# hsinnan75/Dart

Hardware: AMD Instinct MI355X
Metric: M paired-end reads/sec (2x101 bp vs GRCh38-sized index), host to host; records bit-identical to CPU dart (higher is better)
Workload: dtype u64/u8 integer

## Files before the change

dart_amd/csrc/dg_api.hip:

```cpp
#include "../../include/dartgpu.h"
#include "dg_common.h"
#include "dg_fm.h"
#include "dg_seedq.h"
#include "dg_chain.h"
#include "dg_report.h"
#include "dg_pair.h"
#include "dg_reseed.h"
#include "dg_sort.h"
#include "dg_samfmt.h"
#include <stdio.h>
#include <stdlib.h>
#include <string.h>
#include <string>
#include <algorithm>
#include <vector>
#include <atomic>
#include <mutex>
#include <chrono>
#include <thread>
#include <condition_variable>
#include <fcntl.h>
#include <unistd.h>
#include <sys/stat.h>

// ... 282 lines not shown
{
    if (!c->env_blocking_sync || !c->ev_wait) return hipStreamSynchronize(c->stream);
    const hipError_t e = hipEventRecord(c->ev_wait, c->stream);
    return e != hipSuccess ? e : hipEventSynchronize(c->ev_wait);
}

#ifdef DG_PROFILE_CLASSES
__device__ unsigned long long g_class_cycles[DG_COST_CLASSES + 1], g_class_chunks[DG_COST_CLASSES + 1];
#endif
template <int MINW>
__global__ void __launch_bounds__(64, MINW)
k_report(const DIndex ix, const DParams pr, int n_reads, int paired, const unsigned char *__restrict__ seq,
         const uint32_t *__restrict__ seq_off, const uint16_t *__restrict__ rlen, const uint32_t *__restrict__ seed_off,
         const DJob *__restrict__ jobs, DCand *__restrict__ cands,
         const uint32_t *__restrict__ rep_off, DSeed *__restrict__ work, const unsigned long long *__restrict__ items,
         const uint32_t *__restrict__ n_items_p, dg_report_out *__restrict__ reports, uint32_t *cigpool, uint32_t cigcap,
         unsigned int *tops, unsigned char *ws, const WSLayout L, unsigned long long *ctr, int *err)
{
    const unsigned long long t_wave0 = wall_clock64();
    const int lane = blockIdx.x * blockDim.x + threadIdx.x;
    __shared__ uint32_t lds_pm[64 * PM_LDS_WORDS];
    if (*err >= DG_ABORT) return;
    LaneCtx cx;
#ifdef DG_PROFILE_CLASSES
    __shared__ unsigned long long ph_acc[DG_NCLS * DG_NPHASE], cls_acc[2 * DG_NCLS];
    for (int q = threadIdx.x; q < DG_NCLS * DG_NPHASE; q += 64) ph_acc[q] = 0;
    for (int q = threadIdx.x; q < 2 * DG_NCLS; q += 64) cls_acc[q] = 0;
    __syncthreads();
    cx.ph = ph_acc;
#endif
    cx.lds = lds_pm + (threadIdx.x & 63) * PM_LDS_WORDS;
    cx.ix = &ix; cx.pr = &pr; cx.L = &L;
    cx.ws = ws + (size_t)lane * L.stride;
    cx.n_nw = cx.nw_cells = cx.n_reseed = cx.reseed_w = 0;
    const unsigned int lo = 0u, hi = *n_items_p;
    unsigned int *next = tops + TOP_REPORT_MAIN;
    while (true) {
        unsigned int ticket = 0;
        if ((threadIdx.x & 63) == 0) ticket = atomicAdd(next, 1u);
        ticket = (unsigned int)__shfl((int)ticket, 0, 64);
        const unsigned int base = lo + ticket * 64u;
        if (base >= hi) break;
        const unsigned int idx = base + (threadIdx.x & 63);
        const bool valid = idx < hi;
        const unsigned long long item = valid ? items[idx] : 0ull;
        const int r = (int)(item >> 32);
        const uint32_t ci = (uint32_t)item, rep_i = valid ? rep_off[r] + (ci - seed_off[r]) : 0u;
        DRead rd;
        rd.sub_score = 0; rd.mis_num = 0; rd.mapq = 0;
        cx.seq = seq + seq_off[r]; cx.rlen = rlen[r];
#ifdef DG_PROFILE_CLASSES
        const long long t_begin = clock64();
        cx.cls = (int)(cands[(uint32_t)items[base]].final_n & 31); cx.t_last = t_begin;
#endif
        d_gen_mapping_report(cx, valid, paired ? (r & 1) == 0 : true, rd, cands + ci, valid ? 1 : 0, jobs, work,
                             reports + rep_i, rep_i, cigpool, tops + 0, cigcap, err, 0, 1, true);
#ifdef DG_PROFILE_CLASSES
        if ((threadIdx.x & 63) == 0) { cls_acc[cx.cls] += (unsigned long long)(clock64() - t_begin); cls_acc[DG_NCLS + cx.cls] += 1ull; }
#endif
    }
#ifdef DG_PROFILE_CLASSES
    __syncthreads();
    for (int q = threadIdx.x; q < DG_NCLS * DG_NPHASE; q += 64) if (ph_acc[q]) atomicAdd(&g_phase[q / DG_NPHASE][q % DG_NPHASE], ph_acc[q]);
    if (threadIdx.x < DG_NCLS && cls_acc[DG_NCLS + threadIdx.x]) { atomicAdd(&g_class_cycles[threadIdx.x], cls_acc[threadIdx.x]); atomicAdd(&g_class_chunks[threadIdx.x], cls_acc[DG_NCLS + threadIdx.x]); }
#endif
    d_wave_add(ctr + CTR_NW, cx.n_nw);
    d_wave_add(ctr + CTR_NWCELLS, cx.nw_cells);
// ... 604 lines not shown
    k_unpack<<<(unsigned)((nw + 255) / 256), 256, 0, c->stream>>>(c->packed_in.p, (uint32_t)nw, W2, 1.0 / (double)W2, rlen_all, rlen ? c->rlen.p : nullptr, c->seq.p, c->seq_off.p, c->rlen.p, c->enc.p, c->d_input_bad);
    if (n_n) {
        k_unpack_n<<<(unsigned)((n_n + 255) / 256), 256, 0, c->stream>>>(c->nlist_in.p, (uint32_t)n_n, W2, (uint32_t)(nw * 16), c->seq.p, c->enc.p, c->d_input_bad);
        HIPCHK(hipMemcpyAsync(&c->h_tail->input_bad, c->d_input_bad, 4, hipMemcpyDeviceToHost, c->stream));
    } else c->h_tail->input_bad = 0;
    HIPCHK(hipGetLastError());
    return DG_OK;
}

extern "C" int dg_batch_upload_packed(dg_ctx *c, int n_reads, int rlen_all, const uint16_t *rlen, int words_per_read, const uint32_t *words, const uint32_t *nlist, size_t n_n)
{
    const int rc = enqueue_upload_packed(c, n_reads, rlen_all, rlen, words_per_read, words, nlist, n_n);
    if (rc) return rc;
    HIPCHK(hipStreamSynchronize(c->stream));
    return DG_OK;
}

extern "C" void *dg_host_alloc(size_t bytes)
{
    void *p = nullptr;
    return hipHostMalloc(&p, bytes ? bytes : 1, hipHostMallocDefault) == hipSuccess ? p : nullptr;
}
extern "C" void dg_host_free(void *p) { if (p) (void)hipHostFree(p); }

static WSLayout make_ws_layout(int R)
{
    WSLayout L;
    auto al = [](uint32_t x) { return (x + 15u) & ~15u; };
    uint32_t o = 0;
    const uint32_t nmax = 2u * (uint32_t)R + 32u;
    L.max_rlen = (uint32_t)R;
    L.cig_off = o; L.cig_cap = 4u * (uint32_t)R + 64u; o = al(o + L.cig_cap * 4u);
    L.nwbits_off = o; L.nwbits_words = ((uint32_t)R + 1u) * ((nmax + 7u) / 8u); o = al(o + L.nwbits_words * 4u);
    L.rows_off = o; L.row_cap = (uint32_t)R + 8u; o = al(o + 2u * L.row_cap * 4u);
    L.str_off = o; L.str_cap = al(3u * (uint32_t)R + 64u); o = al(o + 6u * L.str_cap);
    L.kmer_off = o; L.kmer_cap = (uint32_t)R + 8u > 48u ? (uint32_t)R + 8u : 48u; o = al(o + L.kmer_cap * 8u);
    uint32_t rd = 64; while (rd < (uint32_t)R + 1u) rd <<= 1;
    L.ring_diag = rd; L.ring_words = ((uint32_t)R + 64u) / 64u; L.ring_off = o; o = al(o + rd * L.ring_words * 8u);
    L.stride = (o + 255u) & ~255u;
    return L;
}

#define DG_MAX_DEVICES 64
static std::mutex g_lds_mu;
static size_t g_lds_set[2][DG_MAX_DEVICES];
static hipError_t raise_dynamic_lds(const void *fn, int which, int device, size_t lds)
{
    std::lock_guard<std::mutex> lk(g_lds_mu);
    size_t &cur = g_lds_set[which][device & (DG_MAX_DEVICES - 1)];
    if (lds <= cur) return hipSuccess;
    const hipError_t e = hipFuncSetAttribute(fn, hipFuncAttributeMaxDynamicSharedMemorySize, (int)lds);
    if (e == hipSuccess) cur = lds;
    return e;
}

static hipError_t launch_seed(dg_ctx *c, int n, int H, hipEvent_t after_encode = nullptr)
{
    const int W = 2 * ((c->max_rlen + 15) / 16 > 0 ? (c->max_rlen + 15) / 16 : 1);
    hipError_t e = c->enc.ensure((size_t)W * n + 16);
    if (e != hipSuccess) return e;
    int lg = 0;
    while ((1 << lg) < W / 2) lg++;
    if (!c->enc_ready) k_encode<<<(unsigned)((((size_t)n << lg) + 255) / 256), 256, 0, c->stream>>>(c->seq.p, c->seq_off.p, c->rlen.p, n, W, lg, c->enc.p);
    if (after_encode) { e = hipEventRecord(after_encode, c->stream); if (e != hipSuccess) return e; }
    if ((e = c->seed_heavy.ensure((size_t)n + 16)) != hipSuccess) return e;
    unsigned blocks = (unsigned)c->n_cu * (unsigned)c->env_seed_waves;
// ... 791 lines not shown
        k_chain_rules<<<c->n_cu * 4, 64, 0, c->stream>>>(0, c->seed_off.p, c->cands.p, c->ncand.p, c->heavy.p, c->d_tops + TOP_HEAVY_UNITS, c->chain_picks.p, c->chain_todo.p, c->d_err);
        const TileScan ts = make_tile_scan(c, scan_tiles_seed(n), c->d_tops + TOP_TICKET_PAIR, 2);
        k_pair<false><<<(unsigned)((n + PU_THREADS - 1) / PU_THREADS), PU_THREADS, 0, c->stream>>>(
            c->ix, c->pr, n, 0, 0, 1, c->seq.p, c->seq_off.p, c->enc.p, 1, c->rlen.p, c->seed_off.p, c->seeds.p, c->cands.p, c->ncand.p, c->rep_off.p,
            c->slow_units.p, c->reads_out.p, c->reports.p, c->cigfinal.p, 0xFFFFFFFFu, 0xFFFFFFFFu, ts, c->d_sizes, c->d_tops + TOP_CIG, c->d_ctr, c->d_err, CompactOut{nullptr, nullptr, nullptr, nullptr});
        HIPCHK(hipGetLastError());
        k_batch_end<<<1, 256, 0, c->stream>>>(c->d_sizes, c->d_err, c->d_tops, c->d_ctr, c->h_tail);
        HIPCHK(hipGetLastError());
        c->state_zeroed = true;
        HIPCHK(hipStreamSynchronize(c->stream));
        total = c->h_tail->sizes.total_seeds;
        if (c->h_tail->err == DG_E_SEEDS && attempt < 3) { c->cap_seeds = (size_t)total + total / 4 + 1024; continue; }
        if (c->h_tail->err) { snprintf(c->err, 512, "dg_probe_seeds: device status %d", c->h_tail->err); return DG_ERR_INTERNAL; }
        break;
    }
    if (used) *used = total;
    if (total > cap) return DG_ERR_CAPACITY;
    std::vector<SKey> h(total);
    HIPCHK(hipMemcpyAsync(seed_off, c->seed_off.p, ((size_t)n + 1) * 4, hipMemcpyDeviceToHost, c->stream));
    if (total) HIPCHK(hipMemcpyAsync(h.data(), c->seeds.p, (size_t)total * sizeof(SKey), hipMemcpyDeviceToHost, c->stream));
    HIPCHK(hipStreamSynchronize(c->stream));
    for (uint32_t i = 0; i < total; i++) { rpos[i] = sk_rpos(h[i]); slen[i] = sk_rlen(h[i]); gpos[i] = sk_gpos(h[i]); }
    return DG_OK;
}

__global__ void __launch_bounds__(64)
k_probe_nw(int n, const uint32_t *a_off, const uint32_t *b_off, const char *a, const char *b, const uint32_t *out_off,
           uint32_t *out_len, char *out_a, char *out_b, unsigned char *ws, const WSLayout L, const DIndex ix, const DParams pr)
{
    const int i = blockIdx.x * blockDim.x + threadIdx.x;
    if (i >= n) return;
    LaneCtx cx;
    cx.ix = &ix; cx.pr = &pr; cx.L = &L; cx.ws = ws + (size_t)i * L.stride; cx.seq = nullptr; cx.rlen = 0; cx.lds = nullptr;
    cx.n_nw = cx.nw_cells = cx.n_reseed = cx.reseed_w = 0;
    out_len[i] = (uint32_t)d_nw(cx, a + a_off[i], (int)(a_off[i + 1] - a_off[i]), b + b_off[i], (int)(b_off[i + 1] - b_off[i]), out_a + out_off[i], out_b + out_off[i]);
}
__global__ void __launch_bounds__(64)
k_probe_nw_strips(int n, const uint32_t *a_off, const uint32_t *b_off, const char *a, const char *b, const uint32_t *out_off,
                  uint32_t *out_len, char *out_a, char *out_b, const DIndex ix, const DParams pr)
{
    __shared__ uint32_t lds_pm[64 * PM_LDS_WORDS];
    const int i = blockIdx.x * blockDim.x + threadIdx.x;
    if (i >= n) return;
    LaneCtx cx;
    cx.ix = &ix; cx.pr = &pr; cx.L = nullptr; cx.ws = nullptr; cx.seq = nullptr; cx.rlen = 0; cx.lds = lds_pm + (threadIdx.x & 63) * PM_LDS_WORDS;
    cx.n_nw = cx.nw_cells = cx.n_reseed = cx.reseed_w = 0;
    const char *pa = a + a_off[i], *pb = b + b_off[i];
    const int m = (int)(a_off[i + 1] - a_off[i]), nn = (int)(b_off[i + 1] - b_off[i]);
    uint64_t w[6] = {0, 0, 0, 0, 0, 0};
    for (int k = 0; k < m; k++) w[k >> 3] |= (uint64_t)(unsigned char)pa[k] << ((k & 7) << 3);
    for (int k = 0; k < nn; k++) w[3 + (k >> 3)] |= (uint64_t)(unsigned char)pb[k] << ((k & 7) << 3);
    PairStr ps; ps.A0 = w[0]; ps.A1 = w[1]; ps.A2 = w[2]; ps.B0 = w[3]; ps.B1 = w[4]; ps.B2 = w[5];
    ColList cl;
    d_pair_nw(cx, m, nn, ps, cl);
    char *oa = out_a + out_off[i], *ob = out_b + out_off[i];
    int x = 0, y = 0;
    for (int p_ = 0; p_ < cl.K; p_++) {
        const uint32_t ty = d_colcode(cl, p_) & 3u;
        oa[p_] = ty == 1 ? '-' : pa[x++];
        ob[p_] = ty == 2 ? '-' : pb[y++];
    }
    out_len[i] = (uint32_t)cl.K;
}
__global__ void __launch_bounds__(64)
k_probe_nw_wave(int n, int all_wide, const uint32_t *a_off, const uint32_t *b_off, const char *a, const uint32_t *out_off,
                uint32_t *out_len, char *out_a, char *out_b, unsigned char *ws, const WSLayout L, const DIndex ix, const DParams pr)
{
    const int i = blockIdx.x * blockDim.x + threadIdx.x, lane = threadIdx.x & 63;
    const bool has = i < n;
    LaneCtx cx;
    cx.ix = &ix; cx.pr = &pr; cx.L = &L; cx.ws = ws + (size_t)(has ? i : 0) * L.stride; cx.seq = nullptr; cx.rlen = 0; cx.lds = nullptr;
    cx.n_nw = cx.nw_cells = cx.n_reseed = cx.reseed_w = 0;
    const int m = has ? (int)(a_off[i + 1] - a_off[i]) : 0, nn = has ? (int)(b_off[i + 1] - b_off[i]) : 0;
    const unsigned char *pa = (const unsigned char *)a + (has ? a_off[i] : 0);
    const int64_t gPos = has ? (int64_t)b_off[i] : 0;
    d_nw_wave(cx, has, pa, m, gPos, nn, lane, all_wide != 0);
    if (has) {
        char *g = ws_str(cx, 0);
        d_ref_fill(ix, gPos, nn, g);
        out_len[i] = (uint32_t)d_tb_traceback(cx, (const char *)pa, m, g, nn, out_a + out_off[i], out_b + out_off[i]);
    }
}

struct DevTmp {
    std::vector<void *> ptrs;
    hipError_t alloc(void **p, size_t bytes) { hipError_t e = hipMalloc(p, bytes ? bytes : 16); if (e == hipSuccess) ptrs.push_back(*p); return e; }
    ~DevTmp() { for (void *p : ptrs) (void)hipFree(p); }
};

extern "C" int dg_probe_nw_mode(dg_ctx *c, int mode, int n, const uint32_t *a_off, const uint32_t *b_off, const char *a, const char *b,
                                uint32_t *out_off, uint32_t *out_len, char *out_a, char *out_b, size_t cap)
{
    if (!c || n < 0 || mode < 0 || mode > 3) return DG_ERR_ARG;
    HIPCHK(hipSetDevice(c->device));
    if (n == 0) return DG_OK;
    size_t tot = 0; int mx = 32;
    for (int i = 0; i < n; i++) {
        const int m = (int)(a_off[i + 1] - a_off[i]), nn = (int)(b_off[i + 1] - b_off[i]);
        out_off[i] = (uint32_t)tot; tot += (size_t)m + nn;
        if (m > mx) mx = m;
        if ((nn + 1) / 2 > mx) mx = (nn + 1) / 2;
        if (mode == 1 && (m > PM_MAX || nn > PM_MAX || m < 1 || nn < 1)) { snprintf(c->err, 512, "dg_probe_nw_mode 1: pair %d is not within %d x %d", i, PM_MAX, PM_MAX); return DG_ERR_ARG; }
    }
    if (tot > cap) return DG_ERR_CAPACITY;
    const size_t la = a_off[n], lb = b_off[n];
// ... 43 lines not shown
```

dart_amd/csrc/dg_common.h:

```cpp
#pragma once
#include <hip/hip_runtime.h>
#include <stdint.h>

#define DG_WAVE 64

__host__ __device__ __forceinline__ uint64_t d_u64(uint32_t lo, uint32_t hi) { return ((uint64_t)hi << 32) | lo; }

struct __attribute__((aligned(8))) DSeed {
    int64_t  gPos;
    int32_t  rPos;
    int32_t  rLen;
    int32_t  gLen;
    uint32_t flags;
};
#define SEED_SIMPLE   1u
#define SEED_ACCEPTOR 2u

typedef uint64_t SKey;
__host__ __device__ __forceinline__ SKey sk_make(int64_t gPos, int rPos, int rLen) { return ((uint64_t)gPos << 24) | ((uint64_t)(uint32_t)rPos << 12) | (uint64_t)(uint32_t)rLen; }
__host__ __device__ __forceinline__ int64_t sk_gpos(SKey k) { return (int64_t)(k >> 24); }
__host__ __device__ __forceinline__ int sk_rpos(SKey k) { return (int)((k >> 12) & 0xFFFu); }
__host__ __device__ __forceinline__ int sk_rlen(SKey k) { return (int)(k & 0xFFFu); }
__host__ __device__ __forceinline__ int64_t sk_diag(SKey k) { return sk_gpos(k) - sk_rpos(k); }

// ... 39 lines not shown
    const int64_t  *loc_key;
    const int32_t  *loc_chr;
    const int64_t  *chr_off;
    uint64_t primary, L2[5], seq_len;
    int64_t  l_pac;
    int32_t  n_chr, sa_intv;
    int32_t  ktab_k, sa_dense_intv;
    int32_t  sa_dense_shift;
};

struct DParams {
    int32_t max_gaps, max_dup, max_intron, min_intron, max_mismatch, multi_hit, all_sj, paired;
};

#define DG_E_CIGAR 1
#define DG_E_SJ 2
#define DG_E_JOBS 3
#define DG_ABORT 10
#define DG_E_SEEDS 10
#define DG_E_REPORTS 11
#define DG_E_WORK 12
#define DG_E_CIGFINAL 13
#define DG_E_SCAN 14
#define DG_E_SEEDQ 15
#define DG_COST_CLASSES 32
struct DSizes { uint32_t total_seeds, total_rep, total_work, total_cig, total_sj, n_jobs, n_slow_units, n_heavy_units, cig_fast, pad[3];
                unsigned long long scan_dbg[16]; };

enum { CTR_STEPS = 0, CTR_BLOCKS, CTR_LF, CTR_SA, CTR_SEEDS, CTR_CANDS, CTR_NW, CTR_NWCELLS, CTR_RESEED, CTR_RESEEDW,
       CTR_STEPS_ACT, CTR_BLOCKS_ACT, CTR_KTAB, CTR_LF_ACT, CTR_DIRECT, CTR_MAXTRIPS, CTR_WTRIPS_MAX, CTR_WTRIPS_SUM,
       CTR_RESEED_TRIPS, CTR_RESEED_TICKS,
       CTR_SQ_TRIPS, CTR_SQ_LANES = CTR_SQ_TRIPS + 5, CTR_SQ_PHASES = CTR_SQ_LANES + 5,
       CTR_WT_SEEDQF, CTR_WT_SEEDH, CTR_WT_CHAIN, CTR_WT_PAIR, CTR_WT_REPORT, CTR_R4_N ,
       CTR_RESEED_WHOLE = CTR_R4_N , CTR_RESEED_ITEMS , CTR_RESEED_POOLED , CTR_N };

__host__ __device__ __forceinline__ uint8_t d_nt4(unsigned char c)
{
    const uint32_t u = c & 0xDFu;
    const uint32_t code = ((u >> 1) ^ (u >> 2)) & 3u;
    const bool acgt = (u == 0x41u) | (u == 0x43u) | (u == 0x47u) | (u == 0x54u);
    return (uint8_t)(acgt ? code : (c == '-' ? 5u : 4u));
}

__host__ __device__ __forceinline__ char d_refchar(const DIndex &ix, int64_t g)
{
    const int64_t L = ix.l_pac;
    if (g < 0 || g >= 2 * L) return 0;
    const bool rev = g >= L;
    const int64_t f = rev ? 2 * L - 1 - g : g;
    const uint32_t c = (ix.pac[f >> 2] >> ((~f & 3) << 1)) & 3u;
    return (char)((rev ? 0x41434754u : 0x54474341u) >> (8u * c));
}

typedef uint2 __attribute__((aligned(1))) uint2_a1;
typedef uint32_t __attribute__((aligned(1))) uint32_a1;

__host__ __device__ __forceinline__ uint64_t d_ref8(const DIndex &ix, int64_t g0)
{
    const int64_t L = ix.l_pac;
    uint64_t out = 0;
    if (g0 >= 0 && g0 + 8 <= L) {
        const uint32_t w = __builtin_bswap32(*(const uint32_a1 *)(ix.pac + (g0 >> 2))) << ((g0 & 3) << 1);
#pragma unroll
        for (int k = 0; k < 8; k++) out |= (uint64_t)((0x54474341u >> (8u * ((w >> (30 - 2 * k)) & 3u))) & 0xFFu) << (8 * k);
        return out;
    }
    if (g0 >= L && g0 + 8 <= 2 * L) {
// ... 52 lines not shown
```

dart_amd/csrc/dg_report.h:

```cpp
#pragma once
#include "dg_common.h"

struct WSLayout {
    uint32_t cig_off, cig_cap;
    uint32_t nwbits_off, nwbits_words;
    uint32_t rows_off, row_cap;
    uint32_t str_off, str_cap;
    uint32_t kmer_off, kmer_cap;
    uint32_t ring_off, ring_diag, ring_words;
    uint32_t stride;
    uint32_t max_rlen;
};

struct LaneCtx {
#ifdef DG_PROFILE_CLASSES
    int cls; long long t_last; unsigned long long *ph;
#endif
    uint32_t *lds;
    const DIndex *ix;
    const DParams *pr;
    const unsigned char *seq;
    int rlen;
    unsigned char *ws;
    const WSLayout *L;
    unsigned long long n_nw, nw_cells, n_reseed, reseed_w;
};

#define OP_M 0u
#define OP_I 1u
#define OP_D 2u
#define OP_N 3u
#define OP_S 4u
#define CIG(len, op) ((((uint32_t)(len)) << 4) | (op))

__host__ __device__ __forceinline__ uint32_t *ws_cig(LaneCtx &cx) { return (uint32_t *)(cx.ws + cx.L->cig_off); }
__host__ __device__ __forceinline__ char *ws_str(LaneCtx &cx, int i) { return (char *)(cx.ws + cx.L->str_off + (uint32_t)i * cx.L->str_cap); }

__host__ __device__ __forceinline__ int d_tr2(int v2) { return (int)(((unsigned)v2 + ((unsigned)v2 >> 31)) & ~1u); }
__host__ __device__ __forceinline__ int d_max3(int a, int b, int c) { const int m = a > b ? a : b; return m > c ? m : c; }

#define NW_STRIP 8
__host__ __device__ inline int d_nw(LaneCtx &cx, const char *a, int m, const char *b, int n, char *oa, char *ob)
{
    uint32_t *bits = (uint32_t *)(cx.ws + cx.L->nwbits_off);
    int *colS = (int *)(cx.ws + cx.L->rows_off), *colR = colS + cx.L->row_cap;
    const int nstrips = (n + NW_STRIP - 1) / NW_STRIP;
    cx.n_nw++; cx.nw_cells += (unsigned long long)m * (unsigned long long)n;
    for (int st = 0; st < nstrips; st++) {
        const int j0 = st * NW_STRIP + 1;
        const bool first = st == 0, last = st == nstrips - 1;
        int sp[NW_STRIP], tp[NW_STRIP];
        uint8_t cb[NW_STRIP];
#pragma unroll
        for (int q = 0; q < NW_STRIP; q++) {
            const int j = j0 + q;
            sp[q] = -2 - j; tp[q] = -131072;
            cb[q] = j <= n ? d_nt4((unsigned char)b[j - 1]) : 7;
        }
        int diag0 = first ? 0 : -2 - (j0 - 1);
        int nxtS = 0, nxtR = 0;
        if (!first && m > 0) { nxtS = colS[1]; nxtR = colR[1]; }
        for (int i = 1; i <= m; i++) {
            int left_s, left_r;
            if (first) { left_s = -2 - i; left_r = -131072; }
            else {
                left_s = nxtS; left_r = nxtR;
                if (i < m) { nxtS = colS[i + 1]; nxtR = colR[i + 1]; }
            }
            const uint8_t ca = d_nt4((unsigned char)a[i - 1]);
            int diag = diag0;
            diag0 = left_s;
            uint32_t acc = 0;
#pragma unroll
            for (int q = 0; q < NW_STRIP; q++) {
                int x = left_r - 1, y = left_s - 3;
                const int r = x > y ? x : y;
                x = tp[q] - 1; y = sp[q] - 3;
// ... 621 lines not shown
        if (cn > 0 && i >= 1 && i <= m) {
            int left_s, left_r, diag;
            if (k == 0) { left_s = -2 - i; left_r = -131072; diag = i == 1 ? 0 : -2 - (i - 1); }
            else { left_s = nl_cur_s; left_r = nl_cur_r; diag = i == 1 ? -2 - (j_first - 1) : nl_prev_s; }
            const uint32_t ca = d_nt4(a_cur);
            const int sh = ((i - 1) & 15) << 1;
            int new_prev = prev_s;
#pragma unroll
            for (int q = 0; q < 8; q++) {
                if (q >= cmax) break;
                if (q < cn) {
                    int x = left_r - 1, y = left_s - 3;
                    const int r = x > y ? x : y;
                    x = up_t[q] - 1; y = up_s[q] - 3;
                    const int tt = x > y ? x : y;
                    const int sv = d_tr2(d_max3(diag + (ca == ((cbp >> (4 * q)) & 15u) ? 3 : -3), r, tt));
                    acc[q] |= ((sv == r ? 1u : 0u) | (sv == tt ? 2u : 0u)) << sh;
                    diag = up_s[q];
                    new_prev = diag;
                    up_s[q] = sv; up_t[q] = tt;
                    left_s = sv; left_r = r;
                }
            }
            prev_s = new_prev; cur_s = left_s; cur_r = left_r;
            if (sh == 30 || i == m) {
#pragma unroll
                for (int q = 0; q < 8; q++) if (q < cn) { tb[(size_t)(j_first + q - 1) * RW + ((i - 1) >> 4)] = acc[q]; acc[q] = 0; }
            }
        }
    }
    __syncthreads();
}

__device__ inline void d_nw_wave(LaneCtx &cx, bool has, const unsigned char *a, int m, int64_t gPos, int n, int lane, bool all_wide = false)
{
    if (!__ballot(has)) return;
    const DIndex &ix = *cx.ix;
    const unsigned long long ap = (unsigned long long)a, wp = (unsigned long long)cx.ws;
    unsigned long long todo = __ballot(has && n <= NWG_MAXN && !all_wide);
    while (todo) {
        int own = -1;
        for (int q = 0; q < 64 / 8; q++) {
            const int b = todo ? __ffsll((long long)todo) - 1 : -1;
            if (q == (lane >> 3)) own = b;
            todo &= todo - 1;
        }
        const int src = own < 0 ? 0 : own;
        const unsigned long long a_o = ((unsigned long long)(uint32_t)__shfl((int)(ap >> 32), src, 64) << 32) | (uint32_t)__shfl((int)ap, src, 64);
        const unsigned long long w_o = ((unsigned long long)(uint32_t)__shfl((int)(wp >> 32), src, 64) << 32) | (uint32_t)__shfl((int)wp, src, 64);
        const unsigned long long g_o = ((unsigned long long)(uint32_t)__shfl((int)((unsigned long long)gPos >> 32), src, 64) << 32) | (uint32_t)__shfl((int)gPos, src, 64);
        const int m_o = __shfl(m, src, 64), n_o = __shfl(n, src, 64);
        d_nw_group<8>(ix, own >= 0, (const unsigned char *)a_o, m_o, (int64_t)g_o, n_o, (unsigned char *)w_o, *cx.L, lane);
    }
    todo = __ballot(has && n > NWG_MAXN && n <= NWG_MAXN16 && !all_wide);
    while (todo) {
        int own = -1;
        for (int q = 0; q < 64 / 16; q++) {
            const int b = todo ? __ffsll((long long)todo) - 1 : -1;
            if (q == (lane >> 4)) own = b;
            todo &= todo - 1;
        }
        const int src = own < 0 ? 0 : own;
        const unsigned long long a_o = ((unsigned long long)(uint32_t)__shfl((int)(ap >> 32), src, 64) << 32) | (uint32_t)__shfl((int)ap, src, 64);
        const unsigned long long w_o = ((unsigned long long)(uint32_t)__shfl((int)(wp >> 32), src, 64) << 32) | (uint32_t)__shfl((int)wp, src, 64);
        const unsigned long long g_o = ((unsigned long long)(uint32_t)__shfl((int)((unsigned long long)gPos >> 32), src, 64) << 32) | (uint32_t)__shfl((int)gPos, src, 64);
        const int m_o = __shfl(m, src, 64), n_o = __shfl(n, src, 64);
        d_nw_group<16>(ix, own >= 0, (const unsigned char *)a_o, m_o, (int64_t)g_o, n_o, (unsigned char *)w_o, *cx.L, lane);
    }
    todo = __ballot(has && (n > NWG_MAXN16 || all_wide));
    while (todo) {
        const int owner = __ffsll((long long)todo) - 1;
        todo &= todo - 1;
        const unsigned long long a_o = ((unsigned long long)(uint32_t)__shfl((int)(ap >> 32), owner, 64) << 32) | (uint32_t)__shfl((int)ap, owner, 64);
        const unsigned long long w_o = ((unsigned long long)(uint32_t)__shfl((int)(wp >> 32), owner, 64) << 32) | (uint32_t)__shfl((int)wp, owner, 64);
        const unsigned long long g_o = ((unsigned long long)(uint32_t)__shfl((int)((unsigned long long)gPos >> 32), owner, 64) << 32) | (uint32_t)__shfl((int)gPos, owner, 64);
        const int m_o = __shfl(m, owner, 64), n_o = __shfl(n, owner, 64);
        d_nw_coop(ix, (const unsigned char *)a_o, m_o, (int64_t)g_o, n_o, (unsigned char *)w_o, *cx.L, lane);
    }
}

__host__ __device__ inline int d_tb_traceback(LaneCtx &cx, const char *a, int m, const char *b, int n, char *oa, char *ob)
{
    const uint32_t *tb = (const uint32_t *)(cx.ws + cx.L->nwbits_off);
    const int RW = (m + 15) >> 4;
    cx.n_nw++; cx.nw_cells += (unsigned long long)m * (unsigned long long)n;
    int i = m, j = n, k = 0;
    while (i > 0 || j > 0) {
        uint32_t fl;
        if (i == 0) fl = 1;
        else if (j == 0) fl = 2;
        else fl = (tb[(size_t)(j - 1) * RW + ((i - 1) >> 4)] >> (((i - 1) & 15) << 1)) & 3u;
        if (fl & 1u) { oa[k] = '-'; ob[k] = b[j - 1]; j--; }
        else if (fl & 2u) { oa[k] = a[i - 1]; ob[k] = '-'; i--; }
        else { oa[k] = a[i - 1]; ob[k] = b[j - 1]; i--; j--; }
        k++;
    }
    for (int p = 0, q = k - 1; p < q; p++, q--) {
        char c = oa[p]; oa[p] = oa[q]; oa[q] = c;
        c = ob[p]; ob[p] = ob[q]; ob[q] = c;
    }
    return k;
}
// ... 322 lines not shown
    if (have_tb && cx.lds && !d_has_dash(cx.seq + sp.rPos, sp.rLen)) return d_process_pair_tb(cx, sp, mode, cig, nc);
    char *g = ws_str(cx, 0);
    d_ref_fill(ix, sp.gPos, sp.gLen, g);
    if (sp.rLen == sp.gLen) {
        int n = 0;
        for (int i = 0; i < sp.rLen; i++) if (rd[i] != g[i]) n++;
        if (n <= 2 && n <= (int)(sp.rLen * 0.2)) { cig[nc++] = CIG(sp.rLen, OP_M); return sp.rLen - n; }
    }
    char *o1 = ws_str(cx, 1), *o2 = ws_str(cx, 3);
    int len = have_tb ? d_tb_traceback(cx, rd, sp.rLen, g, sp.gLen, o1, o2) : d_nw(cx, rd, sp.rLen, g, sp.gLen, o1, o2);
    if (mode == 2) return d_add_cigar(o1, o2, len, cig, nc);
    if (!d_local_quality(o1, o2, len)) { cig[nc++] = CIG(sp.rLen, OP_S); return 0; }
    if (mode == 0) {
        int p = 0;
        while (p < len && o1[p] == '-') p++;
        if (p > 0) { o1 += p; o2 += p; len -= p; sp.gPos += p; sp.gLen -= p; }
        p = 0;
        while (p < len && o2[p] == '-') p++;
        if (p > 0) { o1 += p; o2 += p; len -= p; sp.rPos += p; sp.rLen -= p; cig[nc++] = CIG(p, OP_S); }
        return d_add_cigar(o1, o2, len, cig, nc);
    }
    int p = len - 1, c = 0;
    while (p >= 0 && o1[p] == '-') { c++; p--; }
    if (c > 0) { len -= c; sp.gLen -= c; }
    p = len - 1; c = 0;
    while (p >= 0 && o2[p] == '-') { c++; p--; }
    if (c > 0) { len -= c; sp.rLen -= c; }
    const int score = d_add_cigar(o1, o2, len, cig, nc);
    if (c > 0) cig[nc++] = CIG(c, OP_S);
    return score;
}

#ifdef DG_PROFILE_CLASSES
#define DG_NPHASE 12
#define DG_NCLS 33
__device__ unsigned long long g_phase[DG_NCLS][DG_NPHASE];
#define PH(k) do { if ((threadIdx.x & 63) == 0) { const long long t_now = clock64(); cx.ph[cx.cls * DG_NPHASE + (k)] += (unsigned long long)(t_now - cx.t_last); cx.t_last = t_now; } } while (0)
#else
#define PH(k) do { } while (0)
#endif
#define CIG_SLOT 8
struct DRead {
    int score, sub_score, mis_num, mapq, CanNum, iBest;
};

template <typename ReportT>
__device__ inline void d_gen_mapping_report(LaneCtx &cx, bool valid, bool first, DRead &rd, DCand *cands, int ncand, const DJob *jobs,
                                            DSeed *work, ReportT *rep, uint32_t rep_index0, uint32_t *cigpool, unsigned int *cigtop, uint32_t cigcap, int *err,
                                            int cstart = 0, int cstride = 1, bool park = false)
{
    const DIndex &ix = *cx.ix;
    const int lane = threadIdx.x & 63;
    rd.score = rd.iBest = 0;
    if (!valid) ncand = 0;
    rd.CanNum = ncand > 0 ? ncand : 1;
    if (valid && ncand == 0 && cstart == 0) {
        ReportT rp;
        rp.aln_score = 0; rp.sj_type = -1; rp.flag = 0; rp.paired_idx = -1; rp.chr = -1; rp.bdir = 0;
        rp.pos = 0; rp.cigar_off = 0; rp.n_cigar = 0;
        rep[0] = rp;
    }
    int nmax = ncand > cstart ? (ncand - cstart + cstride - 1) / cstride : 0;
    for (int o = 32; o > 0; o >>= 1) { const int v = __shfl_xor(nmax, o, 64); nmax = v > nmax ? v : nmax; }
    uint32_t *cig = ws_cig(cx);
    PH(0);
    for (int it = 0; it < nmax; it++) {
        const int i = cstart + it * cstride;
        const bool act = i < ncand;
        ReportT rp;
        rp.aln_score = 0; rp.sj_type = -1; rp.flag = 0; rp.paired_idx = -1; rp.chr = -1; rp.bdir = 0; rp.pos = 0;
        rp.cigar_off = 0; rp.n_cigar = 0;
        int final_n = 0, num = 0, nq = 0, bigj = -1, npl = 0;
        bool lane_nw_before = false;
        uint32_t nwj = 0;
        uint64_t pcl = 0;
        DSeed *s = work;
        bool go = false, live = false;
        int n = 0;
        if (act) {
            DCand &c = cands[i];
            rp.paired_idx = c.PairedIdx;
            if (c.Score != 0) {
                live = true;
                s = work + c.work_off;
                n = c.n_a;
                const int n0 = n;
                for (int q = 0; q < c.job_count; q++) {
                    const DJob jb = jobs[c.job_first + q];
                    if (jb.found == 1) {
                        DSeed ns; ns.gPos = jb.gPos; ns.rPos = jb.rPos; ns.rLen = ns.gLen = jb.len; ns.flags = SEED_SIMPLE;
                        s[n++] = ns;
                    } else if (jb.found < 0) {
                        DSeed ns;
                        if (d_reseed(cx, jb.rBegin, jb.rBegin + jb.rl, jb.Lb, jb.Lb + jb.glen, &ns)) s[n++] = ns;
                    }
                }
                if (n > n0) d_insertion_sort_seeds(s, n);
            }
        }
        PH(1);
        n = d_seed_extension_wave(cx, live, s, n, lane);
        PH(2);
        if (live) {
            {
                DCand &c = cands[i];
                int2 *vec = (int2 *)(s + n + 1);
                rp.sj_type = c.SJtype = d_check_splice(cx, s, n, vec);
                PH(3);
                n = d_identify_normal_pairs(s, n);
                final_n = num = n;
                go = !(num > 1 && !d_check_coordinate_validity(ix, s, num));
                PH(4);
                if (go) {
                    for (int j = 0; j < num; j++) {
                        const DSeed &sd = s[j];
                        if ((sd.rLen == 0 && sd.gLen == 0) || (sd.flags & SEED_SIMPLE) || j > 254) continue;
                        const int mode = j == 0 ? 0 : (j == num - 1 ? 1 : 2);
                        if (sd.rLen > PM_MAX || sd.gLen > PM_MAX) {
                            if (bigj < 0 && d_big_needs_nw(cx, sd, mode)) { if (sd.gLen <= 64 * 64 && !lane_nw_before) bigj = j; else lane_nw_before = true; }
                            npl++;
                            continue;
                        }
                        PairStr ps; int nm = 0;
                        const int pc = d_pair_classify(cx, sd, mode, ps, nm);
                        if (pc == PC_GENERIC) lane_nw_before = true;
                        if (npl < 12) pcl |= (uint64_t)(pc | ((pc == PC_EQUAL ? nm : 0) << 3)) << (5 * npl);
                        npl++;
                        if (nq < PM_MAXQ && pc == PC_NW) {
                            uint64_t *pin = (uint64_t *)(cx.ws + cx.L->kmer_off) + 16 + 6 * nq;
                            pin[0] = ps.A0; pin[1] = ps.A1; pin[2] = ps.A2; pin[3] = ps.B0; pin[4] = ps.B1; pin[5] = ps.B2;
                            nwj |= (uint32_t)j << (8 * nq); nq++;
                        }
                    }
                }
            }
        }
        PH(5);
        if (__ballot(bigj >= 0)) {
            const DSeed sd = s[bigj < 0 ? 0 : bigj];
            d_nw_wave(cx, bigj >= 0, cx.seq + sd.rPos, sd.rLen, sd.gPos, sd.gLen, lane);
        }
        PH(6);
        if (act && go) {
            int nc = 1, mis_num = 0, aln = 0;
            uint64_t *pmres = (uint64_t *)(cx.ws + cx.L->kmer_off);
            for (int q = 0; q < nq; q++) {
                const int j = (int)((nwj >> (8 * q)) & 255u);
                PairStr ps; ColList cl;
                const uint64_t *pin = pmres + 16 + 6 * q;
                ps.A0 = pin[0]; ps.A1 = pin[1]; ps.A2 = pin[2]; ps.B0 = pin[3]; ps.B1 = pin[4]; ps.B2 = pin[5];
                d_pair_nw(cx, s[j].rLen, s[j].gLen, ps, cl);
                pmres[4 * q] = cl.w0; pmres[4 * q + 1] = cl.w1; pmres[4 * q + 2] = cl.w2; pmres[4 * q + 3] = (uint64_t)cl.K;
            }
            PH(7);
            int qn = 0, pi = 0;
            for (int j = 0; j < num; j++) {
                DSeed &sd = s[j];
                if (sd.rLen == 0 && sd.gLen == 0) continue;
                int g;
                if (j > 0 && (g = (int)(sd.gPos - (s[j - 1].gPos + s[j - 1].gLen))) > 0) cig[nc++] = CIG(g, OP_N);
                if (sd.flags & SEED_SIMPLE) { cig[nc++] = CIG(sd.rLen, OP_M); aln += sd.rLen; }
                else {
                    const int mode = j == 0 ? 0 : (j == num - 1 ? 1 : 2);
                    int score;
                    if (j == bigj) score = d_process_pair(cx, sd, mode, cig, nc, true);
                    else if (qn < nq && (int)((nwj >> (8 * qn)) & 255u) == j) {
                        ColList cl; cl.w0 = pmres[4 * qn]; cl.w1 = pmres[4 * qn + 1]; cl.w2 = pmres[4 * qn + 2]; cl.K = (int)pmres[4 * qn + 3];
                        qn++;
                        score = d_pair_finish(cl, sd, mode, cig, nc);
                    } else {
                        PairStr ps; int nm = 0, pc;
                        const int slot = j > 254 ? 99 : pi;
                        if (slot < 12 && ((pcl >> (5 * slot)) & 7u) != PC_NW) { pc = (int)((pcl >> (5 * slot)) & 7u); nm = (int)((pcl >> (5 * slot + 3)) & 3u); }
                        else pc = d_pair_classify(cx, sd, mode, ps, nm);
                        if (pc == PC_EQUAL) { cig[nc++] = CIG(sd.rLen, OP_M); score = sd.rLen - nm; }
                        else if (pc == PC_ONE) { cx.n_nw++; cx.nw_cells += 1; cig[nc++] = CIG(1, OP_M); score = 0; }
                        else if (pc == PC_NW) { ColList cl; d_pair_nw(cx, sd.rLen, sd.gLen, ps, cl); score = d_pair_finish(cl, sd, mode, cig, nc); }
                        else score = d_process_pair(cx, sd, mode, cig, nc);
                    }
                    if (j <= 254) pi++;
                    aln += score;
                    mis_num += sd.rLen - score;
                }
            }
            PH(8);
            int c0 = 1;
            if (num > 0) {
                int j;
                if ((j = s[0].rPos) > 0) { cig[0] = CIG(j, OP_S); c0 = 0; }
                if ((j = cx.rlen - (s[num - 1].rPos + s[num - 1].rLen)) > 0) cig[nc++] = CIG(j, OP_S);
            }
            if (mis_num > cx.pr->max_mismatch || nc - c0 == 0) aln = 0;
            for (int j = c0; j < nc; j++) if ((cig[j] & 15u) == OP_N && (int)(cig[j] >> 4) < cx.pr->min_intron) { aln = 0; break; }
            if (aln > 0) {
                const int64_t gPos = s[0].gPos, end_gPos = s[num - 1].gPos + s[num - 1].gLen - 1;
                const int lb = d_loc_lower_bound(ix, gPos);
                rp.chr = ix.loc_chr[lb];
                if (gPos < ix.l_pac) { rp.bdir = first ? 1 : 0; rp.pos = gPos + 1 - ix.chr_off[rp.chr]; }
                else { rp.bdir = first ? 0 : 1; rp.pos = ix.loc_key[lb] - end_gPos + 1; }
                if (rp.pos <= 0) aln = 0;
                else {
                    if (gPos >= ix.l_pac) for (int a = c0, b = nc - 1; a < b; a++, b--) { const uint32_t t = cig[a]; cig[a] = cig[b]; cig[b] = t; }
                    int m = 0, cnt = 0;
                    uint32_t state = 99;
                    for (int j = c0; j < nc; j++) {
                        const uint32_t op = cig[j] & 15u, ln = cig[j] >> 4;
                        if (op != state) { if (cnt > 0) cig[m++] = CIG(cnt, state); cnt = (int)ln; state = op; }
                        else cnt += (int)ln;
                    }
                    if (cnt > 0) cig[m++] = CIG(cnt, state);
                    const unsigned int off = m <= CIG_SLOT ? (rep_index0 + (unsigned int)i) * CIG_SLOT : atomicAdd(cigtop, (unsigned int)m);
                    if (off + (unsigned int)m > cigcap) { atomicMax(err, DG_E_CIGAR); rp.n_cigar = 0; }
                    else { for (int j = 0; j < m; j++) cigpool[off + j] = cig[j]; rp.cigar_off = off; rp.n_cigar = (uint32_t)m; }
                }
                rp.aln_score = aln;
                if (cstride != 1 || park) rp.flag = mis_num;
                else if (aln > rd.score) { rd.iBest = i; rd.mis_num = mis_num; rd.sub_score = rd.score; rd.score = aln; }
// ... 52 lines not shown
```

dart_amd/host.py:

```python
from __future__ import annotations

import ctypes as C
import os

import numpy as np

_HERE = os.path.dirname(os.path.abspath(__file__))
LIB_PATH = os.environ.get("DARTGPU_LIB") or os.path.join(_HERE, "libdartgpu.so")


class IndexView(C.Structure):
    _fields_ = [("bwt", C.c_void_p), ("bwt_words", C.c_uint64), ("primary", C.c_uint64), ("L2", C.c_uint64 * 5),
                ("seq_len", C.c_uint64), ("sa", C.c_void_p), ("n_sa", C.c_uint64), ("sa_intv", C.c_int32),
                ("pac", C.c_void_p), ("l_pac", C.c_int64), ("n_chr", C.c_int32), ("chr_off", C.c_void_p),
                ("chr_len", C.c_void_p)]


class Params(C.Structure):
    _fields_ = [(n, C.c_int32) for n in ("max_gaps", "max_dup", "max_intron", "min_intron", "max_mismatch",
                                          "multi_hit", "all_sj", "paired")]


READ_OUT = np.dtype([("score", "<i4"), ("sub_score", "<i4"), ("mis_num", "<i4"), ("mapq", "<i4"), ("n_rep", "<i4"),
                     ("best", "<i4"), ("rep_off", "<i4"), ("sj_off", "<i4"), ("n_sj", "<i4")])
# ... 438 lines not shown

    def device_records_compact(self):
        import torch
        ptrs = (C.c_void_p * 4)(); counts = (C.c_size_t * 4)()
        self._chk(self.lib.dg_batch_device_records_compact(self.ctx, ptrs, counts), "dg_batch_device_records_compact")
        out = []
        for k, item in enumerate((READ_C.itemsize, REPORT_C.itemsize, 4, SJ_OUT.itemsize)):
            nbytes = int(counts[k]) * item

            class _View:
                pass
            v = _View()
            if nbytes == 0 or not ptrs[k]:
                out.append(torch.empty(0, dtype=torch.uint8, device="cuda"))
                continue
            v.__cuda_array_interface__ = {"shape": (nbytes,), "typestr": "|u1", "data": (int(ptrs[k]), False), "version": 2}
            out.append(torch.as_tensor(v, device="cuda"))
        return out

    def timings(self):
        names = (C.c_char_p * 16)()
        ms = (C.c_float * 16)()
        n = self.lib.dg_last_timings(self.ctx, names, ms, 16)
        return [(names[i].decode(), float(ms[i])) for i in range(n)]

    def counters(self):
        out = (C.c_uint64 * 64)()
        n = self.lib.dg_last_counters(self.ctx, out, 64)
        keys = ["steps", "occ_blocks", "lf_steps", "sa_lookups", "seeds", "candidates", "nw_calls", "nw_cells", "reseed_calls", "reseed_window",
                "steps_executed", "occ_blocks_executed", "ktab_lookups", "lf_steps_executed", "direct_extensions", "k_seed_max_trips_per_read", "k_seed_wave_trips_max", "k_seed_wave_trips_sum", "k_reseed_trips", "k_reseed_wave_ticks_100mhz",
                "seedq_trips_begin", "seedq_trips_step", "seedq_trips_compare", "seedq_trips_locate", "seedq_trips_refill",
                "seedq_slots_begin", "seedq_slots_step", "seedq_slots_compare", "seedq_slots_locate", "seedq_slots_refill", "seedq_phases",
                "wave_ticks_k_seed_qf", "wave_ticks_k_seed_heavy", "wave_ticks_k_chain_heavy", "wave_ticks_k_pair", "wave_ticks_k_report", "general_path_units", "wave_chained_units", "batch_runs", "reruns_capacity_total", "reruns_scan_total",
                "k_reseed_windows_scanned_again_whole", "k_reseed_items", "k_reseed_chunks_through_pool"]
        return {keys[i]: int(out[i]) for i in range(min(n, len(keys)))}

    def probe_seeds(self, seq_off, rlen, flat):
        n = len(rlen)
        a, b, c = np.ascontiguousarray(seq_off, np.uint32), np.ascontiguousarray(rlen, np.uint16), np.ascontiguousarray(flat, np.uint8)
        cap = max(1024, n * 64)
        while True:
            so = np.zeros(n + 1, np.uint32); rp = np.zeros(cap, np.int32); sl = np.zeros(cap, np.int32); gp = np.zeros(cap, np.int64)
            used = C.c_size_t(0)
            rc = self.lib.dg_probe_seeds(self.ctx, n, a.ctypes.data, b.ctypes.data, c.ctypes.data, so.ctypes.data, rp.ctypes.data,
                                         sl.ctypes.data, gp.ctypes.data, cap, C.byref(used))
            if rc == -4:
                cap = int(used.value) + 16
                continue
            self._chk(rc, "dg_probe_seeds")
            u = int(used.value)
            return so, rp[:u], sl[:u], gp[:u]

    def probe_nw(self, pairs, mode: int = 0):
        n = len(pairs)
        a_off = np.zeros(n + 1, np.uint32); b_off = np.zeros(n + 1, np.uint32)
        for i, (x, y) in enumerate(pairs):
            a_off[i + 1] = a_off[i] + len(x); b_off[i + 1] = b_off[i] + len(y)
        a = np.frombuffer(b"".join(p[0] for p in pairs) + b"\0", dtype=np.uint8).copy()
        b = np.frombuffer(b"".join(p[1] for p in pairs) + b"\0", dtype=np.uint8).copy()
        cap = int(a_off[n]) + int(b_off[n]) + 16
        out_off = np.zeros(n + 1, np.uint32); out_len = np.zeros(n + 1, np.uint32)
        oa = np.zeros(cap, np.uint8); ob = np.zeros(cap, np.uint8)
        self._chk(self.lib.dg_probe_nw_mode(self.ctx, mode, n, a_off.ctypes.data, b_off.ctypes.data, a.ctypes.data, b.ctypes.data, out_off.ctypes.data,
                                            out_len.ctypes.data, oa.ctypes.data, ob.ctypes.data, cap), "dg_probe_nw_mode")
        res = []
        for i in range(n):
            o, l = int(out_off[i]), int(out_len[i])
# ... 3 lines not shown
```

Baseline: 1172.

## Sort wave NW jobs by size and let big gaps align behind generic pairs

Replaces the ffs-based assignment of lanes to grouped NW jobs with a bitonic sort by cell count, or a popcount prefix placement when few jobs exist. Owner lanes are published through LDS so that similar-sized problems share a pass. The rule for sending a large gap to the wave-wide NW is loosened: it is no longer skipped just because a generic pair came earlier in the same read. The change also adds a separate NW traceback bit buffer in the workspace, a counter for the new case, and profiling sub-phases. The sort adds shuffles and a __syncthreads inside d_nw_wave, and the per-lane workspace grows.

```diff
diff --git a/dart_amd/csrc/dg_api.hip b/dart_amd/csrc/dg_api.hip
--- a/dart_amd/csrc/dg_api.hip
+++ b/dart_amd/csrc/dg_api.hip
@@ -338,7 +338,7 @@
     cx.lds = lds_pm + (threadIdx.x & 63) * PM_LDS_WORDS;
     cx.ix = &ix; cx.pr = &pr; cx.L = &L;
     cx.ws = ws + (size_t)lane * L.stride;
-    cx.n_nw = cx.nw_cells = cx.n_reseed = cx.reseed_w = 0;
+    cx.n_nw = cx.nw_cells = cx.n_reseed = cx.reseed_w = 0; cx.ctr_big_behind = d_ctr_stripe(ctr) + CTR_BIG_WAVE_BEHIND;
     const unsigned int lo = 0u, hi = *n_items_p;
     unsigned int *next = tops + TOP_REPORT_MAIN;
     while (true) {
@@ -1009,6 +1009,7 @@
     L.max_rlen = (uint32_t)R;
     L.cig_off = o; L.cig_cap = 4u * (uint32_t)R + 64u; o = al(o + L.cig_cap * 4u);
     L.nwbits_off = o; L.nwbits_words = ((uint32_t)R + 1u) * ((nmax + 7u) / 8u); o = al(o + L.nwbits_words * 4u);
+    L.nw1bits_off = o; o = al(o + L.nwbits_words * 4u);
     L.rows_off = o; L.row_cap = (uint32_t)R + 8u; o = al(o + 2u * L.row_cap * 4u);
     L.str_off = o; L.str_cap = al(3u * (uint32_t)R + 64u); o = al(o + 6u * L.str_cap);
     L.kmer_off = o; L.kmer_cap = (uint32_t)R + 8u > 48u ? (uint32_t)R + 8u : 48u; o = al(o + L.kmer_cap * 8u);
@@ -1866,7 +1867,7 @@
     if (i >= n) return;
     LaneCtx cx;
     cx.ix = &ix; cx.pr = &pr; cx.L = &L; cx.ws = ws + (size_t)i * L.stride; cx.seq = nullptr; cx.rlen = 0; cx.lds = nullptr;
-    cx.n_nw = cx.nw_cells = cx.n_reseed = cx.reseed_w = 0;
+    cx.n_nw = cx.nw_cells = cx.n_reseed = cx.reseed_w = 0; cx.ctr_big_behind = nullptr;
     out_len[i] = (uint32_t)d_nw(cx, a + a_off[i], (int)(a_off[i + 1] - a_off[i]), b + b_off[i], (int)(b_off[i + 1] - b_off[i]), out_a + out_off[i], out_b + out_off[i]);
 }
 __global__ void __launch_bounds__(64)
@@ -1878,7 +1879,7 @@
     if (i >= n) return;
     LaneCtx cx;
     cx.ix = &ix; cx.pr = &pr; cx.L = nullptr; cx.ws = nullptr; cx.seq = nullptr; cx.rlen = 0; cx.lds = lds_pm + (threadIdx.x & 63) * PM_LDS_WORDS;
-    cx.n_nw = cx.nw_cells = cx.n_reseed = cx.reseed_w = 0;
+    cx.n_nw = cx.nw_cells = cx.n_reseed = cx.reseed_w = 0; cx.ctr_big_behind = nullptr;
     const char *pa = a + a_off[i], *pb = b + b_off[i];
     const int m = (int)(a_off[i + 1] - a_off[i]), nn = (int)(b_off[i + 1] - b_off[i]);
     uint64_t w[6] = {0, 0, 0, 0, 0, 0};
@@ -1902,9 +1903,10 @@
 {
     const int i = blockIdx.x * blockDim.x + threadIdx.x, lane = threadIdx.x & 63;
     const bool has = i < n;
+    __shared__ uint32_t lds_pm[64 * PM_LDS_WORDS];
     LaneCtx cx;
-    cx.ix = &ix; cx.pr = &pr; cx.L = &L; cx.ws = ws + (size_t)(has ? i : 0) * L.stride; cx.seq = nullptr; cx.rlen = 0; cx.lds = nullptr;
-    cx.n_nw = cx.nw_cells = cx.n_reseed = cx.reseed_w = 0;
+    cx.ix = &ix; cx.pr = &pr; cx.L = &L; cx.ws = ws + (size_t)(has ? i : 0) * L.stride; cx.seq = nullptr; cx.rlen = 0; cx.lds = lds_pm + lane * PM_LDS_WORDS;
+    cx.n_nw = cx.nw_cells = cx.n_reseed = cx.reseed_w = 0; cx.ctr_big_behind = nullptr;
     const int m = has ? (int)(a_off[i + 1] - a_off[i]) : 0, nn = has ? (int)(b_off[i + 1] - b_off[i]) : 0;
     const unsigned char *pa = (const unsigned char *)a + (has ? a_off[i] : 0);
     const int64_t gPos = has ? (int64_t)b_off[i] : 0;
diff --git a/dart_amd/csrc/dg_common.h b/dart_amd/csrc/dg_common.h
--- a/dart_amd/csrc/dg_common.h
+++ b/dart_amd/csrc/dg_common.h
@@ -95,7 +95,8 @@
        CTR_RESEED_TRIPS, CTR_RESEED_TICKS,
        CTR_SQ_TRIPS, CTR_SQ_LANES = CTR_SQ_TRIPS + 5, CTR_SQ_PHASES = CTR_SQ_LANES + 5,
        CTR_WT_SEEDQF, CTR_WT_SEEDH, CTR_WT_CHAIN, CTR_WT_PAIR, CTR_WT_REPORT, CTR_R4_N ,
-       CTR_RESEED_WHOLE = CTR_R4_N , CTR_RESEED_ITEMS , CTR_RESEED_POOLED , CTR_N };
+       CTR_RESEED_WHOLE = CTR_R4_N , CTR_RESEED_ITEMS , CTR_RESEED_POOLED ,
+       CTR_BIG_WAVE_BEHIND , CTR_N };
 
 __host__ __device__ __forceinline__ uint8_t d_nt4(unsigned char c)
 {
diff --git a/dart_amd/csrc/dg_report.h b/dart_amd/csrc/dg_report.h
--- a/dart_amd/csrc/dg_report.h
+++ b/dart_amd/csrc/dg_report.h
@@ -4,6 +4,7 @@
 struct WSLayout {
     uint32_t cig_off, cig_cap;
     uint32_t nwbits_off, nwbits_words;
+    uint32_t nw1bits_off;
     uint32_t rows_off, row_cap;
     uint32_t str_off, str_cap;
     uint32_t kmer_off, kmer_cap;
@@ -24,6 +25,7 @@
     unsigned char *ws;
     const WSLayout *L;
     unsigned long long n_nw, nw_cells, n_reseed, reseed_w;
+    unsigned long long *ctr_big_behind;
 };
 
 #define OP_M 0u
@@ -42,7 +44,7 @@
 #define NW_STRIP 8
 __host__ __device__ inline int d_nw(LaneCtx &cx, const char *a, int m, const char *b, int n, char *oa, char *ob)
 {
-    uint32_t *bits = (uint32_t *)(cx.ws + cx.L->nwbits_off);
+    uint32_t *bits = (uint32_t *)(cx.ws + cx.L->nw1bits_off);
     int *colS = (int *)(cx.ws + cx.L->rows_off), *colR = colS + cx.L->row_cap;
     const int nstrips = (n + NW_STRIP - 1) / NW_STRIP;
     cx.n_nw++; cx.nw_cells += (unsigned long long)m * (unsigned long long)n;
@@ -730,42 +732,65 @@
     __syncthreads();
 }
 
+#define NWQ_NONE 0xFFFFFFFFu
+__host__ __device__ __forceinline__ uint32_t d_nwq_key(bool has, int m, int n, int lane)
+{
+    if (!has || n > NWG_MAXN16) return NWQ_NONE;
+    return (n > NWG_MAXN ? 0x80000000u : 0u) | (((uint32_t)m * (uint32_t)n) << 6) | (uint32_t)lane;
+}
+__host__ __device__ __forceinline__ uint32_t d_nwq_cmpx(uint32_t mine, uint32_t other, int lane, int k, int j)
+{
+    const bool ascending = (lane & k) == 0, lower = (lane & j) == 0;
+    const uint32_t lo = mine < other ? mine : other, hi = mine < other ? other : mine;
+    return ascending == lower ? lo : hi;
+}
+__host__ __device__ __forceinline__ int d_nwq_source(int pass, int group, int groups, int first, int count)
+{
+    const int p = pass * groups + group;
+    return p < count ? first + p : -1;
+}
+
+template <int NWG_LANES>
+__device__ inline void d_nw_serve(LaneCtx &cx, int own, unsigned long long ap, unsigned long long wp, int m, int64_t gPos, int n, int lane)
+{
+    const int src = own < 0 ? 0 : own;
+    const unsigned long long a_o = ((unsigned long long)(uint32_t)__shfl((int)(ap >> 32), src, 64) << 32) | (uint32_t)__shfl((int)ap, src, 64);
+    const unsigned long long w_o = ((unsigned long long)(uint32_t)__shfl((int)(wp >> 32), src, 64) << 32) | (uint32_t)__shfl((int)wp, src, 64);
+    const unsigned long long g_o = ((unsigned long long)(uint32_t)__shfl((int)((unsigned long long)gPos >> 32), src, 64) << 32) | (uint32_t)__shfl((int)gPos, src, 64);
+    const int m_o = __shfl(m, src, 64), n_o = __shfl(n, src, 64);
+    d_nw_group<NWG_LANES>(*cx.ix, own >= 0, (const unsigned char *)a_o, m_o, (int64_t)g_o, n_o, (unsigned char *)w_o, *cx.L, lane);
+}
+
 __device__ inline void d_nw_wave(LaneCtx &cx, bool has, const unsigned char *a, int m, int64_t gPos, int n, int lane, bool all_wide = false)
 {
     if (!__ballot(has)) return;
     const DIndex &ix = *cx.ix;
     const unsigned long long ap = (unsigned long long)a, wp = (unsigned long long)cx.ws;
-    unsigned long long todo = __ballot(has && n <= NWG_MAXN && !all_wide);
-    while (todo) {
-        int own = -1;
-        for (int q = 0; q < 64 / 8; q++) {
-            const int b = todo ? __ffsll((long long)todo) - 1 : -1;
-            if (q == (lane >> 3)) own = b;
-            todo &= todo - 1;
-        }
-        const int src = own < 0 ? 0 : own;
-        const unsigned long long a_o = ((unsigned long long)(uint32_t)__shfl((int)(ap >> 32), src, 64) << 32) | (uint32_t)__shfl((int)ap, src, 64);
-        const unsigned long long w_o = ((unsigned long long)(uint32_t)__shfl((int)(wp >> 32), src, 64) << 32) | (uint32_t)__shfl((int)wp, src, 64);
-        const unsigned long long g_o = ((unsigned long long)(uint32_t)__shfl((int)((unsigned long long)gPos >> 32), src, 64) << 32) | (uint32_t)__shfl((int)gPos, src, 64);
-        const int m_o = __shfl(m, src, 64), n_o = __shfl(n, src, 64);
-        d_nw_group<8>(ix, own >= 0, (const unsigned char *)a_o, m_o, (int64_t)g_o, n_o, (unsigned char *)w_o, *cx.L, lane);
-    }
-    todo = __ballot(has && n > NWG_MAXN && n <= NWG_MAXN16 && !all_wide);
-    while (todo) {
-        int own = -1;
-        for (int q = 0; q < 64 / 16; q++) {
-            const int b = todo ? __ffsll((long long)todo) - 1 : -1;
-            if (q == (lane >> 4)) own = b;
-            todo &= todo - 1;
-        }
-        const int src = own < 0 ? 0 : own;
-        const unsigned long long a_o = ((unsigned long long)(uint32_t)__shfl((int)(ap >> 32), src, 64) << 32) | (uint32_t)__shfl((int)ap, src, 64);
-        const unsigned long long w_o = ((unsigned long long)(uint32_t)__shfl((int)(wp >> 32), src, 64) << 32) | (uint32_t)__shfl((int)wp, src, 64);
-        const unsigned long long g_o = ((unsigned long long)(uint32_t)__shfl((int)((unsigned long long)gPos >> 32), src, 64) << 32) | (uint32_t)__shfl((int)gPos, src, 64);
-        const int m_o = __shfl(m, src, 64), n_o = __shfl(n, src, 64);
-        d_nw_group<16>(ix, own >= 0, (const unsigned char *)a_o, m_o, (int64_t)g_o, n_o, (unsigned char *)w_o, *cx.L, lane);
-    }
-    todo = __ballot(has && (n > NWG_MAXN16 || all_wide));
+    const bool grouped = has && !all_wide;
+    int cnt = __popcll(__ballot(grouped && n <= NWG_MAXN));
+    {
+        const unsigned long long narrow = __ballot(grouped && n <= NWG_MAXN), wide = __ballot(grouped && n > NWG_MAXN && n <= NWG_MAXN16);
+        if (cnt > 64 / 8 || __popcll(wide) > 64 / 16) {
+            uint32_t key = d_nwq_key(grouped, m, n, lane);
+#pragma unroll 1
+            for (int k = 2; k <= 64; k <<= 1)
+#pragma unroll 1
+                for (int j = k >> 1; j > 0; j >>= 1) key = d_nwq_cmpx(key, (uint32_t)__shfl_xor((int)key, j, 64), lane, k, j);
+            cx.lds[0] = key & 63u;
+        } else if (grouped && n <= NWG_MAXN16) {
+            const unsigned long long below = (1ull << lane) - 1ull;
+            const int p = n <= NWG_MAXN ? __popcll(narrow & below) : cnt + __popcll(wide & below);
+            cx.lds[(p - lane) * PM_LDS_WORDS] = (uint32_t)lane;
+        }
+        __syncthreads();
+    }
+    auto owner_at = [&](int p) -> int { return p < 0 ? -1 : (int)cx.lds[(p - lane) * PM_LDS_WORDS]; };
+    for (int t = 0; t * (64 / 8) < cnt; t++)
+        d_nw_serve<8>(cx, owner_at(d_nwq_source(t, lane >> 3, 64 / 8, 0, cnt)), ap, wp, m, gPos, n, lane);
+    cnt = __popcll(__ballot(grouped && n > NWG_MAXN && n <= NWG_MAXN16));
+    for (int t = 0; t * (64 / 16) < cnt; t++)
+        d_nw_serve<16>(cx, owner_at(d_nwq_source(t, lane >> 4, 64 / 16, __popcll(__ballot(grouped && n <= NWG_MAXN)), cnt)), ap, wp, m, gPos, n, lane);
+    unsigned long long todo = __ballot(has && (n > NWG_MAXN16 || all_wide));
     while (todo) {
         const int owner = __ffsll((long long)todo) - 1;
         todo &= todo - 1;
@@ -1154,7 +1179,7 @@
 }
 
 #ifdef DG_PROFILE_CLASSES
-#define DG_NPHASE 12
+#define DG_NPHASE 14
 #define DG_NCLS 33
 __device__ unsigned long long g_phase[DG_NCLS][DG_NPHASE];
 #define PH(k) do { if ((threadIdx.x & 63) == 0) { const long long t_now = clock64(); cx.ph[cx.cls * DG_NPHASE + (k)] += (unsigned long long)(t_now - cx.t_last); cx.t_last = t_now; } } while (0)
@@ -1193,7 +1218,7 @@
         rp.aln_score = 0; rp.sj_type = -1; rp.flag = 0; rp.paired_idx = -1; rp.chr = -1; rp.bdir = 0; rp.pos = 0;
         rp.cigar_off = 0; rp.n_cigar = 0;
         int final_n = 0, num = 0, nq = 0, bigj = -1, npl = 0;
-        bool lane_nw_before = false;
+        int behind = 0;
         uint32_t nwj = 0;
         uint64_t pcl = 0;
         DSeed *s = work;
@@ -1239,13 +1264,13 @@
                         if ((sd.rLen == 0 && sd.gLen == 0) || (sd.flags & SEED_SIMPLE) || j > 254) continue;
                         const int mode = j == 0 ? 0 : (j == num - 1 ? 1 : 2);
                         if (sd.rLen > PM_MAX || sd.gLen > PM_MAX) {
-                            if (bigj < 0 && d_big_needs_nw(cx, sd, mode)) { if (sd.gLen <= 64 * 64 && !lane_nw_before) bigj = j; else lane_nw_before = true; }
+                            if (bigj < 0 && d_big_needs_nw(cx, sd, mode)) { if (sd.gLen <= 64 * 64) { bigj = j; behind <<= 1; } else behind = 1; }
                             npl++;
                             continue;
                         }
                         PairStr ps; int nm = 0;
                         const int pc = d_pair_classify(cx, sd, mode, ps, nm);
-                        if (pc == PC_GENERIC) lane_nw_before = true;
+                        if (pc == PC_GENERIC && bigj < 0) behind = 1;
                         if (npl < 12) pcl |= (uint64_t)(pc | ((pc == PC_EQUAL ? nm : 0) << 3)) << (5 * npl);
                         npl++;
                         if (nq < PM_MAXQ && pc == PC_NW) {
@@ -1259,6 +1284,7 @@
         }
         PH(5);
         if (__ballot(bigj >= 0)) {
+            if (const unsigned long long late = __ballot(behind == 2)) { if (lane == 0 && cx.ctr_big_behind) atomicAdd(cx.ctr_big_behind, (unsigned long long)__popcll(late)); }
             const DSeed sd = s[bigj < 0 ? 0 : bigj];
             d_nw_wave(cx, bigj >= 0, cx.seq + sd.rPos, sd.rLen, sd.gPos, sd.gLen, lane);
         }
@@ -1276,7 +1302,13 @@
             }
             PH(7);
             int qn = 0, pi = 0;
+#ifdef DG_PROFILE_CLASSES
+            for (int part = 0; part < 3; part++) {
+            const int j_lo = part == 0 ? 0 : (bigj < 0 ? (part == 1 ? num : 0) : bigj + part - 1), j_hi = part == 2 ? num : (bigj < 0 ? 0 : bigj + part);
+            for (int j = j_lo; j < j_hi; j++) {
+#else
             for (int j = 0; j < num; j++) {
+#endif
                 DSeed &sd = s[j];
                 if (sd.rLen == 0 && sd.gLen == 0) continue;
                 int g;
@@ -1305,6 +1337,10 @@
                     mis_num += sd.rLen - score;
                 }
             }
+#ifdef DG_PROFILE_CLASSES
+            if (part < 2) PH(11 + part);
+            }
+#endif
             PH(8);
             int c0 = 1;
             if (num > 0) {
diff --git a/dart_amd/host.py b/dart_amd/host.py
--- a/dart_amd/host.py
+++ b/dart_amd/host.py
@@ -494,7 +494,8 @@
                 "seedq_trips_begin", "seedq_trips_step", "seedq_trips_compare", "seedq_trips_locate", "seedq_trips_refill",
                 "seedq_slots_begin", "seedq_slots_step", "seedq_slots_compare", "seedq_slots_locate", "seedq_slots_refill", "seedq_phases",
                 "wave_ticks_k_seed_qf", "wave_ticks_k_seed_heavy", "wave_ticks_k_chain_heavy", "wave_ticks_k_pair", "wave_ticks_k_report", "general_path_units", "wave_chained_units", "batch_runs", "reruns_capacity_total", "reruns_scan_total",
-                "k_reseed_windows_scanned_again_whole", "k_reseed_items", "k_reseed_chunks_through_pool"]
+                "k_reseed_windows_scanned_again_whole", "k_reseed_items", "k_reseed_chunks_through_pool",
+                "large_pairs_aligned_wave_wide_behind_a_string_path_pair"]
         return {keys[i]: int(out[i]) for i in range(min(n, len(keys)))}
 
     def probe_seeds(self, seq_off, rlen, flat):
```

Result: no change. 1182 (median of 6 runs) (+0.8%).
